# kzampog/cilantro

Hardware: AMD Instinct MI355X
Metric: ICP corr. pairs/sec (+ iterations/sec), synthetic uniform clouds (higher is better)
Workload: dtype f32 search / f64 accumulate+solve

## Files before the change

cilantro_amd/build.py:

```python
import os
import subprocess
import sys
from concurrent.futures import ThreadPoolExecutor

HERE = os.path.dirname(os.path.abspath(__file__))
CSRC = os.path.join(HERE, "csrc")
LIBDIR = os.path.join(HERE, "lib")
OBJDIR = os.path.join(HERE, "lib", "obj")
LIB = os.path.join(LIBDIR, "libcilantro_hip.so")
SOURCES = ["kernels.hip", "warm.hip", "epilogue.hip", "affine.hip", "feat_warm.hip", "extract.hip", "grid_build.hip", "grid_downsample.hip", "components.hip", "filters.hip", "kmeans.hip", "ransac.hip", "ransac_transform.hip", "knn.hip", "bidir.hip", "tie_build.hip", "c_api.hip", "icp_loop.hip", "multi.hip"]
HEADERS = ["internal.hpp", "ctx.hpp", "device_mem.hpp", "stateless.hpp", "ransac_sampling.hpp", "loop_policy.hpp", "grid_policy.hpp", "solve.hpp", "rccl_api.hpp", "search_device.hpp", "affine_device.hpp", os.path.join("..", "..", "include", "cilantro_hip", "c_api.h")]
HIPCC = os.environ.get("HIPCC", "/opt/rocm/bin/hipcc")
FLAGS = ["--offload-arch=gfx950", "-O3", "-std=c++17", "-fPIC", "-ffp-contract=off", "-Wall",
         "-Wno-unused-result", "-DNDEBUG"]
EXTRA_FLAGS = {f: ["-fno-slp-vectorize"] for f in ("kernels.hip", "warm.hip", "epilogue.hip", "affine.hip", "extract.hip")}


def _stale(out, deps):
    if not os.path.exists(out):
        return True
    t = os.path.getmtime(out)
    return any(os.path.getmtime(d) > t for d in deps)


def build(force=False, verbose=False, defines=(), tag=""):
    global OBJDIR, LIB
# ... 36 lines not shown
```

cilantro_amd/csrc/c_api.hip:

```cpp
#include <algorithm>
#include <chrono>
#include <cmath>
#include <cstddef>
#include <cstdio>
#include <cstring>
#include <new>

#include "ctx.hpp"
#include "stateless.hpp"

namespace cilhip {
hipStream_t ctx_stream(const cilhip_ctx* c) { return c->stream; }
double ctx_wait_us(const cilhip_ctx* c) { return c->wait_us; }
}

static void drop_src_grid(cilhip_ctx* c) {
  static_cast<SrcGridBufs&>(*c) = SrcGridBufs{};
  c->src_grid = GridDev{}; c->has_src_grid = false;
}
static void drop_feat_tie_tables(cilhip_ctx* c) {
  c->d_tief_leaf_slot.reset(); c->d_tief_nodes.reset();
}
static void drop_tie_tables(cilhip_ctx* c) {
  c->d_tie_leaf_slot.reset(); c->d_tie_nodes.reset();
// ... 13 lines not shown
  if (device < 0 || device >= ndev) return CILHIP_ERR_INVALID;
  cilhip_ctx* c = new (std::nothrow) cilhip_ctx();
  if (!c) return CILHIP_ERR_HIP;
  c->device = device;
  if (hipSetDevice(device) != hipSuccess || c->own_stream.create() != hipSuccess) {
    delete c;
    return CILHIP_ERR_HIP;
  }
  c->stream = c->own_stream;
  if (c->d_state.alloc(1) != hipSuccess || c->d_count.alloc(1) != hipSuccess ||
      c->d_defer_flag.alloc(1) != hipSuccess || hipMemset(c->d_defer_flag, 0, sizeof(uint32_t)) != hipSuccess ||
      c->d_unproven.alloc(128) != hipSuccess || hipMemset(c->d_unproven, 0, 128 * sizeof(uint32_t)) != hipSuccess ||
      c->d_ticket.alloc(1) != hipSuccess || hipMemset(c->d_ticket, 0, sizeof(unsigned int)) != hipSuccess ||
      hipHostMalloc(&c->h_feedback, sizeof(Feedback), hipHostMallocMapped | hipHostMallocCoherent) != hipSuccess ||
      hipHostGetDevicePointer(reinterpret_cast<void**>(&c->d_feedback), c->h_feedback, 0) != hipSuccess ||
      c->d_trace.alloc(RUN_TRACE_CAP) != hipSuccess || hipMemset(c->d_trace, 0, RUN_TRACE_CAP * sizeof(uint4)) != hipSuccess ||
      c->d_stage.alloc(REDUCE_STAGE_DOUBLES) != hipSuccess || c->d_sums.alloc(3 * SUMS_MAX) != hipSuccess) {
    delete c;
    return CILHIP_ERR_HIP;
  }
  if (hipMemset(c->d_state, 0, sizeof(IcpState)) != hipSuccess) { delete c; return CILHIP_ERR_HIP; }
  c->d_tie_counters = reinterpret_cast<unsigned int*>(reinterpret_cast<char*>(c->d_state.get()) + offsetof(IcpState, tie_counters));
  memcpy(c->sort_T, kIdentity16, sizeof(kIdentity16));
  memcpy(c->nn_T, kIdentity16, sizeof(kIdentity16));
  *out = c;
  return CILHIP_OK;
}

static void free_source(cilhip_ctx* c) {
  static_cast<SourceBufs&>(*c) = SourceBufs{};
  c->src_grid = GridDev{}; c->has_src_grid = false;
  c->rev_tie_valid = false; c->rev_tie_aware = false;
  c->src3_valid = false; c->lb_fresh = false; c->rec_valid = false;
  c->d_tiles = nullptr; c->d_tile_center = nullptr; c->ntiles = 0;
  c->has_source = false; c->src_sorted = false; drop_matches(c); c->ns = 0;
  c->have_pairs = false; c->pairs.count = 0;
// ... 192 lines not shown
#ifdef CILHIP_EXP_PHASE_CLOCKS
  cilhip::debug_dump_phase_clocks();
#endif
  return CILHIP_OK;
}

int cilhip_debug_live_allocations(unsigned long long out[2]) {
  if (!out) return CILHIP_ERR_INVALID;
  out[0] = dev_mem_live().count.load(std::memory_order_relaxed);
  out[1] = dev_mem_live().bytes.load(std::memory_order_relaxed);
  return CILHIP_OK;
}

int cilhip_get_last_timing2(cilhip_ctx* c, double* search_ms, double* accumulate_ms) {
  if (!c) return CILHIP_ERR_INVALID;
  if (search_ms) *search_ms = c->last_search_ms;
  if (accumulate_ms) *accumulate_ms = c->last_acc_ms;
  return CILHIP_OK;
}

int cilhip_get_last_iteration_timing(cilhip_ctx* c, int cap, int* n, unsigned int* iteration, float* kernel_ms) {
  if (!c || !n || cap < 0) return CILHIP_ERR_INVALID;
  const size_t m = c->timed_ms.size() < c->timed_iter.size() ? c->timed_ms.size() : c->timed_iter.size();
  *n = (int)m;
  for (size_t k = 0; k < m && k < (size_t)cap; ++k) { if (iteration) iteration[k] = c->timed_iter[k]; if (kernel_ms) kernel_ms[k] = c->timed_ms[k]; }
  return CILHIP_OK;
}

int cilhip_get_last_form_timing(cilhip_ctx* c, int form, double* kernel_ms, int* launches) {
  if (!c || form < 0 || form > 4) return CILHIP_ERR_INVALID;
  if (kernel_ms) *kernel_ms = c->form_ms[form];
  if (launches) *launches = c->form_n[form];
  return CILHIP_OK;
}

int cilhip_get_last_run_trace(cilhip_ctx* c, int cap, int* n_out, unsigned int* unproven, unsigned int* listed, float* step, float* delta, int* form) {
  if (!c || !n_out || cap < 0) return CILHIP_ERR_INVALID;
  CK(c, hipSetDevice(c->device));
  IcpState hs;
  CK(c, hipMemcpyAsync(&hs, c->d_state, sizeof(hs), hipMemcpyDeviceToHost, c->stream));
  uint4 tr[RUN_TRACE_CAP];
  CK(c, hipMemcpyAsync(tr, c->d_trace, sizeof(tr), hipMemcpyDeviceToHost, c->stream));
  CK(c, hipStreamSynchronize(c->stream));
  const int n = std::min(std::min(hs.iterations, (int)RUN_TRACE_CAP), cap);
  for (int i = 0; i < n; ++i) {
// ... 1411 lines not shown

int cilhip_get_grid_info(cilhip_ctx* c, cilhip_grid_info* o) {
  if (!c || !o) return CILHIP_ERR_INVALID;
  if (!c->has_target) return fail(c, CILHIP_ERR_INVALID, "no target");
  o->nx = c->grid.nx; o->ny = c->grid.ny; o->nz = c->grid.nz;
  o->cell = c->grid.cell;
  o->origin[0] = c->grid.ox; o->origin[1] = c->grid.oy; o->origin[2] = c->grid.oz;
  o->n_cells = c->grid_cells;
  o->avg_occupancy = c->grid_occ;
  o->build_ms = c->build_ms;
  return CILHIP_OK;
}

int cilhip_get_last_timing(cilhip_ctx* c, double* loop_ms, double* search_ms, int* launches) {
  if (!c) return CILHIP_ERR_INVALID;
  if (loop_ms) *loop_ms = c->last_loop_ms;
  if (search_ms) *search_ms = c->last_search_ms;
  if (launches) *launches = c->last_search_launches;
  return CILHIP_OK;
}
```

cilantro_amd/csrc/ctx.hpp:

```cpp
#pragma once

#include "../../include/cilantro_hip/c_api.h"

#include <hip/hip_runtime.h>

#include <string>
#include <vector>

#include "internal.hpp"
#include "loop_policy.hpp"

using namespace cilhip;

struct CtxStream { StreamGuard own_stream; };
struct TargetBufs {
  GridStore grid_store;
  SharedBuf<uint32_t> d_inv_perm;
  SharedBuf<uint2> d_tief_leaf_slot;
  SharedBuf<uint4> d_tief_nodes;
  SharedBuf<uint2> d_tie_leaf_slot;
  SharedBuf<uint4> d_tie_nodes;
  SharedBuf<float> d_safe2;
  DevBuf<unsigned long long> d_winner;
  DevBuf<float> d_dst_rgb;
// ... 44 lines not shown
  double build_ms = 0.0;
  float dst_mean[3] = {0, 0, 0};
  uint32_t index_offset = 0;
  bool partial_target = false;

  bool has_source = false;
  uint32_t ns = 0;
  uint2* d_tiles = nullptr;
  float4* d_tile_center = nullptr;
  float tile_axes[9] = {0, 0, 0, 0, 0, 0, 0, 0, 0};
  DevBuf<uint32_t> d_defer_flag;
  DevBuf<uint32_t> d_unproven;
  LoopPolicy policy;
  Feedback* h_feedback = nullptr;
  Feedback* d_feedback = nullptr;
  unsigned int run_tag = 0;
  int last_fused_iters = 0, last_two_pass_iters = 0, last_warm_iters = 0;
  int run_calls = 0;
  std::vector<unsigned char> iter_form;
  std::vector<unsigned char> trace_form;
  double form_ms[5] = {0, 0, 0, 0, 0};
  int form_n[5] = {0, 0, 0, 0, 0};
  int warm_start = 1;
  DevBuf<uint32_t> d_dbg;
  DevBuf<uint4> d_trace;
  uint32_t ntiles = 0;
  int tiled = 1;
  bool src_sorted = false;
  float sort_T[16];
  float src_mean[3] = {0, 0, 0};
// ... 70 lines not shown
  bool have_pairs = false;
  DevBuf<IcpState> d_state_id;

  cilhip_icp_params run_prm{};
  bool run_active = false;
  int guard_axis = -1;
  float guard_slack = 0.0f, guard_center[3] = {0, 0, 0}, guard_half[3] = {0, 0, 0}, guard_T[16] = {0};
  float run_src_mean[3] = {0, 0, 0};

  bool kernel_timing = false;
  int timing_stride = 1;
  std::vector<unsigned int> timed_iter;
  std::vector<float> timed_ms;
  double last_loop_ms = 0.0, last_search_ms = 0.0, last_acc_ms = 0.0;
  int last_search_launches = 0;
  size_t run_nev = 0;
  std::vector<hipEvent_t> ev, ev_acc;
  std::vector<hipEvent_t> ev_ar;
  size_t run_nar = 0;
  double last_allreduce_ms = 0.0; int last_allreduce_n = 0;
  double run_enqueue_us = 0.0; int run_enqueue_iters = 0;
};

inline cilhip_ctx::~cilhip_ctx() {
  if (h_feedback) (void)hipHostFree(h_feedback);
  for (auto e : ev) (void)hipEventDestroy(e);
  for (auto e : ev_acc) (void)hipEventDestroy(e);
  for (auto e : ev_ar) (void)hipEventDestroy(e);
}

#define CK(ctx, call)                                                                                   \
  do {                                                                                                  \
    hipError_t e_ = (call);                                                                             \
    if (e_ != hipSuccess) {                                                                             \
      (ctx)->err = std::string(#call) + ": " + hipGetErrorString(e_);                                   \
      return CILHIP_ERR_HIP;                                                                            \
    }                                                                                                   \
  } while (0)

namespace cilhip {
// ... 42 lines not shown
int ensure_safe2(cilhip_ctx* c);
int ensure_feature_arrays(cilhip_ctx* c);
int ensure_reverse_buffers(cilhip_ctx* c);
void set_warm_args(const cilhip_ctx* c, IterArgs& wa);
CorrWeights corr_weights_of(const cilhip_ctx* c, const cilhip_icp_params* p);
FeatSpec feat_spec_of(const cilhip_ctx* c);
TieDev tie_dev_rev(const cilhip_ctx* c);
int tie_prepare(cilhip_ctx* c, const char* what);
int tie_check_pending(cilhip_ctx* c, bool* again);
int apply_filters(cilhip_ctx* c);
IterArgs make_iter_args(cilhip_ctx* c, float max_sq);
int launch_search(cilhip_ctx* c, const IterArgs& a, int lanes = -1 );
int run_pair_search(cilhip_ctx* c, const IterArgs& a, float max_sq, const float T_host[16]);
int icp_run_affine(cilhip_ctx* c, const cilhip_icp_params* p, const float* T0, cilhip_icp_result* out);
int iter_metric_of(const cilhip_ctx* c, const cilhip_icp_params* p);
}
```

cilantro_amd/csrc/epilogue.hip:

```cpp
#include "search_device.hpp"
#include "affine_device.hpp"

namespace cilhip {

__device__ void reduce_partials_block(const double* __restrict__ partials, int nblocks, double* sums ) {
  __shared__ double sh[4][64];
  const int slot = threadIdx.x & 63, grp = threadIdx.x >> 6;
  double v = 0.0;
  if (slot < SUMS_MAX) {
    int b = grp;
    for (; b + 28 < nblocks; b += 32) {
      double r[8];
#pragma unroll
      for (int k = 0; k < 8; ++k) r[k] = partials[(size_t)(b + 4 * k) * SUMS_MAX + slot];
#pragma unroll
      for (int k = 0; k < 8; ++k) v += r[k];
    }
    for (; b < nblocks; b += 4) v += partials[(size_t)b * SUMS_MAX + slot];
  }
  sh[grp][slot] = v;
  __syncthreads();
  if (threadIdx.x < SUMS_MAX)
    sums[threadIdx.x] = (sh[0][threadIdx.x] + sh[1][threadIdx.x]) + (sh[2][threadIdx.x] + sh[3][threadIdx.x]);
  __syncthreads();
// ... 106 lines not shown

__device__ __forceinline__ void publish_state(const SolveArgs& a, const IcpState& lst) {
  if (a.trace != nullptr && a.gn_last_step && threadIdx.x == 0 && lst.iterations >= 1 && lst.iterations <= RUN_TRACE_CAP)
    a.trace[lst.iterations - 1] = make_uint4(lst.unproven, lst.listed, __float_as_uint(lst.motion_step), __float_as_uint(lst.delta));
  if (a.feedback != nullptr && a.gn_last_step && threadIdx.x == 0) {
    FeedbackSlot* sl = &a.feedback->slot[(unsigned int)lst.iterations & 3u];
    sl->unproven = lst.unproven;
    sl->listed = lst.listed;
    sl->delta = lst.delta;
    sl->prev_delta = lst.prev_delta;
    sl->step = lst.motion_step;
    sl->commit = ((unsigned long long)a.run_tag << 32) | (unsigned long long)(unsigned int)lst.iterations;
    __threadfence_system();
    a.feedback->latest = ((unsigned long long)a.run_tag << 32) | (lst.done ? 0x80000000ull : 0ull) | (unsigned long long)((unsigned int)lst.iterations & 0x7fffffffu);
  }
}

__device__ __forceinline__ void solve_body(const SolveArgs& a) {
  __shared__ double sums[SUMS_MAX];
  __shared__ IcpState lst;
  static_assert(sizeof(IcpState) % 4 == 0, "IcpState is copied as dwords");
  constexpr int ST_DWORDS = (int)(sizeof(IcpState) / 4);
  if (a.state->done) return;
  static_assert(ST_DWORDS <= 256, "one dword of the state per thread");
  const uint32_t sreg = (int)threadIdx.x < ST_DWORDS ? reinterpret_cast<const uint32_t*>(a.state)[threadIdx.x] : 0u;
  __shared__ unsigned int unproven_total;
  __shared__ unsigned int listed_total;
  const bool counters = a.unproven_cnt != nullptr && a.gn_last_step && threadIdx.x < 128;
  unsigned int cv = counters ? a.unproven_cnt[threadIdx.x] : 0u;
  if (a.nblocks > 0) {
// ... 61 lines not shown
        for (int r = 0; r < 3; ++r)
          t[r] = st->dtd[r] - (L[r * 3] * (double)st->smt[0] + L[r * 3 + 1] * (double)st->smt[1] + L[r * 3 + 2] * (double)st->smt[2]) +
                 (double)a.dst_mean[r];
      }
      finalize = true;
    }
  }
  if (finalize) {
    float Tn[16];
    const float delta = compose_update(L, t, st->T, Tn);
    finalize_state(st, a, Tn, delta);
  }
  }
  __syncthreads();
  for (int k = threadIdx.x; k < ST_DWORDS; k += 256) reinterpret_cast<uint32_t*>(a.state)[k] = reinterpret_cast<const uint32_t*>(&lst)[k];
  publish_state(a, lst);
}
__global__ __launch_bounds__(256) void k_solve(SolveArgs a) { solve_body(a); }

void launch_solve(const SolveArgs& a, hipStream_t s) {
  hipLaunchKernelGGL(k_solve, dim3(1), dim3(256), 0, s, a);
}

__global__ __launch_bounds__(256) void k_reduce_solve(const double* __restrict__ partials, int nblocks, double* __restrict__ stage, unsigned int* ticket, SolveArgs a) {
  if (a.state->done) return;
  {
    __shared__ double rsums[SUMS_MAX];
    const int per = (nblocks + (int)gridDim.x - 1) / (int)gridDim.x;
    const int b0 = blockIdx.x * per;
    const int b1 = min(b0 + per, nblocks);
// ... 212 lines not shown
    for (int r = 0; r < 3; ++r) dn = __fadd_rn(dn, __fmul_rn(dT[12 + r], dT[12 + r]));
    const float delta = sqrtf(dn);
    for (int i = 0; i < SUMS_MAX; ++i) st->sums[i] = 0.0;
    st->sums[0] = n;
    finalize_state(st, a, Tn, delta);
#ifdef CILHIP_EXP_AFF_CLOCKS
    {
      const unsigned long long c4_ = wall_clock64();
      st->unproven = (unsigned int)((c1_ - c0_) & 0xffffu) | (unsigned int)(((c2_ - c1_) & 0xffffu) << 16);
      st->listed = (unsigned int)((c3_ - c2_) & 0xffffu) | (unsigned int)(((c4_ - c3_) & 0xffffu) << 16);
    }
#endif
  }
  __syncthreads();
  for (int k = t; k < ST_DWORDS; k += NT) reinterpret_cast<uint32_t*>(a.state)[k] = reinterpret_cast<const uint32_t*>(&lst)[k];
  publish_state(a, lst);
}

void launch_reduce_and_solve_affine(const double* partials, int nrows, double* stage, const SolveArgs& a0, hipStream_t s) {
  SolveArgs a = a0;
  a.gn_last_step = 1;
  if (nrows > 64) {
    hipLaunchKernelGGL(k_reduce_affine, dim3(AFF_GROUPS), dim3(AFF_ROW), 0, s, partials, nrows, stage, (const IcpState*)a.state);
    a.partials = stage; a.nblocks = AFF_GROUPS;
  } else {
    a.partials = partials; a.nblocks = nrows;
  }
  a.reduced = nullptr;
  hipLaunchKernelGGL(k_solve_affine, dim3(1), dim3(AFF_SOLVE_THREADS), 0, s, a);
}
// ... 41 lines not shown
```

cilantro_amd/csrc/icp_loop.hip:

```cpp
#include <algorithm>
#include <chrono>
#include <cmath>
#include <cstddef>
#include <cstring>

#include "ctx.hpp"
#include "rccl_api.hpp"

int cilhip::iter_metric_of(const cilhip_ctx* c, const cilhip_icp_params* p) {
  if (p->metric == CILHIP_METRIC_POINT_TO_POINT) return IM_KABSCH;
  const bool wp = p->w_p2p > 0.0f, wl = p->w_p2pl > 0.0f;
  if (wl && !c->has_normals) return IM_POINT;
  if (wp && wl) return IM_BOTH;
  if (wl) return IM_PLANE;
  if (wp) return IM_POINT;
  return IM_PLANE;
}

static SolveArgs make_solve_args(cilhip_ctx* c, const cilhip_icp_params* p, int im, const float src_mean[3]) {
  SolveArgs sa{};
  sa.state = c->d_state;
  sa.partials = c->d_partials;
  sa.nblocks = iter_num_blocks(c->ns);
  sa.reduced = nullptr;
// ... 32 lines not shown
        v->unproven = sl->unproven; v->listed = sl->listed; v->delta = sl->delta; v->prev_delta = sl->prev_delta; v->step = iters ? sl->step : INFINITY;
        if (iters == 0u || sl->commit == (((unsigned long long)c->run_tag << 32) | iters)) return 0;
      }
    }
    cpu_relax(spins);
    if ((spins & 1023u) == 1023u && std::chrono::duration<double>(std::chrono::steady_clock::now() - t0).count() > patience_s) return 1;
  }
}
static int wait_published_or_sync(cilhip_ctx* c, unsigned int need, FbView* v) {
  if (wait_published(c, need, 30.0, v) == 0) return CILHIP_OK;
  CK(c, hipStreamSynchronize(c->stream));
  if (wait_published(c, need, 0.01, v) == 0) return CILHIP_OK;
  return fail(c, CILHIP_ERR_HIP, "icp_run: the device stopped publishing its loop state");
}

static int read_state(cilhip_ctx* c, cilhip_icp_result* out, float* Tprev = nullptr) {
  IcpState hs;
  CK(c, hipMemcpyAsync(&hs, c->d_state, sizeof(hs), hipMemcpyDeviceToHost, c->stream));
  CK(c, hipStreamSynchronize(c->stream));
  memcpy(c->tie_counters_host, hs.tie_counters, sizeof(c->tie_counters_host));
  c->tie_counters_fresh = true;
  memcpy(out->T, hs.T, sizeof(hs.T));
  if (Tprev) memcpy(Tprev, hs.Tprev, sizeof(hs.Tprev));
  out->iterations = (size_t)hs.iterations;
  out->last_delta_norm = hs.delta;
  out->last_ncorr = (size_t)hs.ncorr;
  return CILHIP_OK;
}

static void finish_run_matches(cilhip_ctx* c, const cilhip_icp_params* p, size_t iterations, const float Tprev[16], bool stored, bool pairs) {
  drop_matches(c); c->have_pairs = false;
  if (iterations == 0) return;
  memcpy(c->nn_T, Tprev, sizeof(c->nn_T));
  if (pairs) { c->have_pairs = true; c->matches_origin = 1; return; }
  if (stored && c->ns) {
    c->have_nn = true; c->d2_stale = true; c->matches_origin = 1;
  } else {
    c->pending_matches = true; c->pending_max_sq = p->max_sq_dist; c->matches_origin = 2;
  }
}

struct RunSetup {
  const cilhip_icp_params* p;
// ... 38 lines not shown
  launch_search_tiled(fa, im, c->d_tiles, c->d_tile_center, c->d_tile_box, c->ntiles, c->stream);
  c->rec_valid = recs; c->lb_fresh = false;
  return recs;
}

static int stop_when_done(cilhip_ctx* c, size_t it, size_t max_iter, bool* stop) {
  *stop = false;
  if (!(max_iter > 64 && (it + 1) % 32 == 0 && it + 1 < max_iter)) return CILHIP_OK;
  int done = 0;
  CK(c, hipMemcpyAsync(&done, reinterpret_cast<const char*>(c->d_state.get()) + offsetof(IcpState, done), sizeof(int), hipMemcpyDeviceToHost, c->stream));
  CK(c, hipStreamSynchronize(c->stream));
  *stop = done != 0;
  return CILHIP_OK;
}

static int finish_run(cilhip_ctx* c, const RunSetup& r, bool stored, bool pairs) {
  CK(c, hipEventRecord(r.e_end, c->stream));
  CK(c, hipGetLastError());
  float Tprev[16];
  const int rc = read_state(c, r.out, Tprev);
  if (rc) return rc;
  finish_run_matches(c, r.p, r.out->iterations, Tprev, stored, pairs && r.out->iterations > 0);
  float ms = 0.f;
  CK(c, hipEventElapsedTime(&ms, r.e_beg, r.e_end));
  c->last_loop_ms = ms; c->last_search_ms = 0.0; c->last_search_launches = 0;
  return CILHIP_OK;
}

static int run_reverse_loop(cilhip_ctx* c, RunSetup& r) {
  const cilhip_icp_params* p = r.p;
  IterArgs& a = r.a;
  SolveArgs& sa = r.sa;
  const int im = r.im;
  int rc = ensure_reverse_buffers(c);
  if (rc) return rc;
  FeatSpec rf = a.feat;
  rf.src = c->src_grid.nrm;
  if (rf.dst2) rf.src2 = c->d_src_rgb_grid;
  if (feat6(c) && (!rf.src || !rf.dst || (rf.dst2 && !rf.src2))) return fail(c, CILHIP_ERR_INVALID, "feature search: both clouds' feature vectors are needed");
  const int nb_f = iter_num_blocks(c->ns), nb_r = iter_num_blocks(c->grid.n);
  const bool fwd_wcap = c->search_dir == 2 && warm_capable(c);
// ... 51 lines not shown
      sa.reduced = nullptr;
      launch_solve(sa, c->stream);
    }
    bool stop = false;
    rc = stop_when_done(c, it, p->max_iter, &stop);
    if (rc) return rc;
    if (stop) break;
  }
  c->last_acc_ms = 0.0;
  return finish_run(c, r, false, false);
}

static int run_pair_list_loop(cilhip_ctx* c, RunSetup& r) {
  const cilhip_icp_params* p = r.p;
  SolveArgs& sa = r.sa;
  for (size_t it = 0; it < p->max_iter; ++it) {
    int rc = run_pair_search(c, r.a, p->max_sq_dist, it == 0 ? r.Ti : r.out->T);
    if (rc) return rc;
    IterArgs pa = r.a;
    pa.nn_d2 = c->pairs.d2;
    pa.src = c->pairs.src_view; pa.src_nrm = (c->d_src_nrm && c->symmetric) ? c->pairs.nrm_view : nullptr; pa.ns = c->pairs.count; pa.nn_pos = c->pairs.posd;
    const int pnb = iter_num_blocks(pa.ns);
    rc = ensure_partial_rows(c, (size_t)pnb);
    if (rc) return rc;
    pa.partials = c->d_partials;
    for (size_t st = 0; st < r.opt_steps; ++st) {
      pa.skip_if_inner_done = (st > 0);
      sa.gn_last_step = (st + 1 == r.opt_steps);
      if (pa.ns) {
        launch_iter(pa, r.im, false, false, pnb, c->stream);
// ... 152 lines not shown
    }
    sa.gn_last_step = (st + 1 == opt_steps);
    if (c->ns) {
      const int prows = (st == 0 && warm) ? warm_num_blocks(c->ns) : (st == 0 && one_pass) ? tiled_partial_rows(c->ntiles) : (st == 0 && feat_fused_it) ? feat_warm_blocks(c->ns)
                        : r.affine ? r.nb_aff : nb;
      if (r.affine) launch_reduce_and_solve_affine(c->d_partials, prows, c->d_stage, sa, c->stream);
      else launch_reduce_and_solve(c->d_partials, prows, c->d_stage, c->fused_epilogue ? c->d_ticket : nullptr, sa, c->stream);
    } else {
      launch_solve(sa, c->stream);
    }
  }
  f.prev_stored = stored_now && c->ns != 0;
  return CILHIP_OK;
}

static int collect_kernel_timing(cilhip_ctx* c, const ForwardRun& f, size_t iterations) {
  size_t executed = 0;
  while (executed < c->timed_iter.size() && (size_t)c->timed_iter[executed] < iterations) ++executed;
  c->last_acc_ms = 0.0;
  c->timed_ms.assign(executed, 0.0f);
  for (size_t k = 0; k < executed; ++k) {
    float m = 0.f;
    CK(c, hipEventElapsedTime(&m, c->ev[2 + 2 * k], c->ev[3 + 2 * k]));
    c->timed_ms[k] = m;
    c->last_search_ms += m;
    if (k < c->iter_form.size()) { c->form_ms[c->iter_form[k]] += m; ++c->form_n[c->iter_form[k]]; }
  }
  for (size_t k = 0; k + 1 < f.nacc; k += 2) {
    float m = 0.f;
    CK(c, hipEventElapsedTime(&m, c->ev_acc[k], c->ev_acc[k + 1]));
    c->last_acc_ms += m;
  }
  c->last_search_launches = (int)executed;
  return CILHIP_OK;
}

static int run_forward_loop(cilhip_ctx* c, RunSetup& r) {
  const cilhip_icp_params* p = r.p;
  IterArgs& a = r.a;
  int rc;
  if (feat6(c)) { rc = ensure_feature_arrays(c); if (rc) return rc; a.feat = feat_spec_of(c); }
  if (!filters_active(c) && !(a.cw.enabled && feat6(c))) a.nn_d2 = nullptr;
  ForwardRun f{};
// ... 5 lines not shown
  f.fwcap = feat6(c) && c->feat_warm && c->warm_start != 0 && c->ns >= 400000 && !filters_active(c) && !c->fused && !r.affine;
  if (f.fwcap) {
    rc = ensure_safe2(c); if (rc) return rc;
    rc = grow_partials(c, r, (size_t)feat_warm_blocks(c->ns)); if (rc) return rc;
  }
  f.paced = ((f.tile_acc || f.wcap) && c->ns && p->max_iter > 2 && c->tile_acc_adaptive) || (f.fwcap && p->max_iter > 2);
  if (f.tile_acc && !c->tile_acc_adaptive) c->policy.far_mode = false;
  c->last_fused_iters = c->last_two_pass_iters = c->last_warm_iters = 0;
  c->rec_valid = false; c->lb_fresh = false;
  c->policy.begin_run(c->warm_enter * c->grid.cell);
  c->iter_form.clear(); c->trace_form.clear(); c->timed_iter.clear();
  for (int k = 0; k < 5; ++k) { c->form_ms[k] = 0.0; c->form_n[k] = 0; }
  f.glanes = c->group_lanes > 0 ? c->group_lanes
             : (c->group_lanes < 0 && !use_tiled(c) && !feat6(c) && !c->fused) ? (c->ns <= 400000u ? 16 : c->ns <= 1500000u ? 8 : 0) : 0;
  f.group_now = f.glanes != 0 && (c->group_lanes > 0 || !f.wcap);
  for (size_t it = 0; it < p->max_iter; ++it) {
    bool stop = false;
    if (f.paced) { rc = pace_forward(c, f, it, &stop); if (rc) return rc; if (stop) break; }
    const bool one_pass = f.tile_acc && !c->policy.far_mode;
    const bool warm = f.wcap && it >= 1 && (c->warm_start == 2 || (f.paced && c->policy.on));
    const bool timing_it = f.timing && (c->timing_stride <= 1 || it < 3 || it % (size_t)c->timing_stride == 0);
    rc = enqueue_forward_iteration(c, r, f, it, one_pass, warm, timing_it);
    if (rc) return rc;
    if (!f.paced) { rc = stop_when_done(c, it, p->max_iter, &stop); if (rc) return rc; if (stop) break; }
  }
  rc = finish_run(c, r, f.all_stored && !filters_active(c) && !feat6(c), false);
  if (rc) return rc;
#ifdef CILHIP_EXP_PHASE_CLOCKS
  cilhip::debug_dump_phase_clocks();
#endif
  return f.timing ? collect_kernel_timing(c, f, r.out->iterations) : CILHIP_OK;
}

static int icp_run_once(cilhip_ctx* c, const cilhip_icp_params* p, const float* T0, cilhip_icp_result* out) {
  if (c->weight_fn && p->metric == CILHIP_METRIC_COMBINED && c->transform_mode == 0) {
    if (c->search_dir != 0) return fail(c, CILHIP_ERR_UNSUPPORTED, "a pair-weight callback runs with SECOND_TO_FIRST searches (rigid loop); estimate from pair lists through cilhip_estimate_combined");
    c->last_loop_ms = 0.0; c->last_search_ms = 0.0; c->last_acc_ms = 0.0; c->last_search_launches = 0;
    return cilhip_icp_run_two_sets(c, p->max_sq_dist, c, p->max_sq_dist, p, T0, out);
  }
  RunSetup r{};
  r.p = p; r.out = out;
  r.affine = c->transform_mode == 1;
  if (r.affine) {
    if (c->index_offset) return fail(c, CILHIP_ERR_UNSUPPORTED, "the affine variants are not available on target shards");
    const bool device_loop = c->affine_device_loop && c->ns != 0 && c->grid.n != 0 && c->search_dir == 0 && !filters_active(c) && !weighted(c) && !feat6(c) && !c->fused &&
                             !(c->d_src_nrm && c->symmetric) && c->guard_axis < 0;
    if (!device_loop) return icp_run_affine(c, p, T0, out);
  }
  r.Ti = T0 ? T0 : kIdentity16;
  int rc = ensure_sorted(c, r.Ti);
  if (rc) return rc;
  const bool affine_combined = r.affine && p->metric == CILHIP_METRIC_COMBINED;
  r.im = !r.affine ? iter_metric_of(c, p) : (affine_combined && p->w_p2pl > 0.0f && c->has_normals) ? IM_AFFC : IM_AFFP;
  r.gn = (r.im != IM_KABSCH) && !r.affine;
  const bool zero_steps = r.gn && p->max_opt_iter == 0;
  r.opt_steps = r.gn ? (p->max_opt_iter ? p->max_opt_iter : 1) : 1;
  ++c->run_tag;
  launch_init_state(c->d_state, r.Ti, c->src_mean, c->stream, c->d_feedback, c->run_tag, c->src_center, c->src_half, c->d_tie_counters);
  if (r.gn && c->ns >= 65536) ensure_pair_records(c);
  r.a = make_iter_args(c, p->max_sq_dist);
  if (!c->pair_records) r.a.grid.pn = nullptr;
  r.a.cw = corr_weights_of(c, p);
  r.sa = make_solve_args(c, p, r.im, c->src_mean);
  r.sa.gn_zero_steps = zero_steps ? 1 : 0;
  r.nb = r.sa.nblocks;
  r.nb_aff = r.affine ? affine_acc_blocks(c->ns) : 0;
  if (r.affine) {
    r.a.no_centering = affine_combined ? 0 : 1;
    r.sa.affine_centered = affine_combined ? 1 : 0;
    if (!affine_combined) { r.sa.w_p2p = 1.0f; r.sa.w_p2pl = 0.0f; }
    const size_t rows = (size_t)std::max(r.nb_aff, warm_num_blocks(c->ns));
    rc = grow_partials(c, r, (rows * AFF_ROW + SUMS_MAX - 1) / SUMS_MAX);
    if (rc) return rc;
  }
  if (c->ns == 0) {
    CK(c, hipMemsetAsync(c->d_sums, 0, SUMS_MAX * sizeof(double), c->stream));
    r.sa.nblocks = 0;
    r.sa.reduced = c->d_sums;
  }
  r.e_beg = event_at(c->ev, 0); r.e_end = event_at(c->ev, 1);
  return c->search_dir != 0 ? run_other_directions(c, r) : run_forward_loop(c, r);
}

int cilhip_icp_run(cilhip_ctx* c, const cilhip_icp_params* p, const float* T0, cilhip_icp_result* out) {
  if (!c || !p || !out) return CILHIP_ERR_INVALID;
  if (p->metric != CILHIP_METRIC_POINT_TO_POINT && p->metric != CILHIP_METRIC_COMBINED) return fail(c, CILHIP_ERR_INVALID, "icp_run: bad metric");
  CK(c, hipSetDevice(c->device));
  int rc = tie_prepare(c, "icp_run");
  if (rc) return rc;
  rc = icp_run_once(c, p, T0, out);
  if (rc) return rc;
  bool again = false;
  rc = tie_check_pending(c, &again);
  if (rc) return rc;
  return again ? icp_run_once(c, p, T0, out) : CILHIP_OK;
}

int cilhip_icp_begin(cilhip_ctx* c, const cilhip_icp_params* p, const float* T0, const float* gmean) {
  if (!c || !p) return CILHIP_ERR_INVALID;
  CK(c, hipSetDevice(c->device));
  if (p->metric == CILHIP_METRIC_COMBINED && p->max_opt_iter != 1) return fail(c, CILHIP_ERR_UNSUPPORTED, "sharded runs support max_opt_iter == 1");
  if (filters_active(c)) return fail(c, CILHIP_ERR_UNSUPPORTED, "inlier_fraction / one_to_one are global filters: not available in sharded runs");
  if (c->weight_fn && p->metric == CILHIP_METRIC_COMBINED)
    return fail(c, CILHIP_ERR_UNSUPPORTED, "a pair-weight callback is evaluated on the host, per estimate: not available in sharded runs (the stock evaluators are)");
  { const int trc = tie_prepare(c, "icp_begin"); if (trc) return trc; }
  if (c->search_dir != 0) return fail(c, CILHIP_ERR_UNSUPPORTED, "search directions other than SECOND_TO_FIRST are not available in sharded runs");
  if (feat6(c) || c->transform_mode != 0) return fail(c, CILHIP_ERR_UNSUPPORTED, "point+normal features and the affine variants are not available in sharded runs");
  const float* Ti = T0 ? T0 : kIdentity16;
  int rc = ensure_sorted(c, Ti);
  if (rc) return rc;
  c->run_prm = *p;
  for (int i = 0; i < 3; ++i) c->run_src_mean[i] = gmean ? gmean[i] : c->src_mean[i];
  ++c->run_tag;
  launch_init_state(c->d_state, Ti, c->run_src_mean, c->stream, c->d_feedback, c->run_tag, c->src_center, c->src_half, c->d_tie_counters);
  CK(c, hipGetLastError());
  c->run_active = true;
  c->run_nev = 0; c->run_nar = 0; c->last_allreduce_ms = 0.0; c->last_allreduce_n = 0;
  c->run_enqueue_us = 0.0; c->run_enqueue_iters = 0;
  c->run_calls = 0;
  c->rec_valid = false; c->lb_fresh = false;
  c->policy.begin_run(c->warm_enter * c->grid.cell);
  if (warm_capable(c) && !(c->d_src_nrm && c->symmetric)) { rc = ensure_safe2(c); if (rc) return rc; rc = ensure_warm_buffers(c); if (rc) return rc; }
  c->iter_form.clear(); c->trace_form.clear();
  for (int k = 0; k < 5; ++k) { c->form_ms[k] = 0.0; c->form_n[k] = 0; }
  c->last_fused_iters = c->last_two_pass_iters = c->last_warm_iters = 0;
  return CILHIP_OK;
}

// ... 207 lines not shown
```

cilantro_amd/csrc/internal.hpp:

```cpp
#pragma once

#include <hip/hip_runtime.h>
#include <stdint.h>

#include <string>
#include <thread>

#include "device_mem.hpp"
#include "grid_policy.hpp"
#include "solve.hpp"

struct cilhip_ctx;

namespace cilhip {

constexpr uint32_t NONE_U32 = 0xFFFFFFFFu;
#ifndef CILHIP_CUBE_EDGE
#define CILHIP_CUBE_EDGE 12
#endif
constexpr int CUBE_EDGE = CILHIP_CUBE_EDGE;
#ifndef CILHIP_TILE_THREADS
#define CILHIP_TILE_THREADS 1024
#endif
#ifndef CILHIP_TILE_WAVES_PER_SIMD
// ... 138 lines not shown
};

struct FeedbackSlot {
  unsigned int unproven;
  unsigned int listed;
  float delta;
  float prev_delta;
  float step;
  float pad;
  unsigned long long commit;
};
struct Feedback {
  FeedbackSlot slot[4];
  unsigned long long latest;
};

struct SolveArgs {
  Feedback* feedback;
  unsigned int run_tag;
  IcpState* state;
  const double* partials;
  int nblocks;
  const double* reduced;
  int metric;
  float w_p2p, w_p2pl;
  int point_weighted;
  float conv_tol, opt_conv_tol;
  float dst_mean[3], src_mean[3];
  int gn_last_step;
  int gn_zero_steps;
  int has_normals;
  int affine_centered;
  uint32_t* unproven_cnt;
  int guard_axis;
  float guard_slack;
  float guard_center[3], guard_half[3];
  float guard_T[16];
  float src_center[3], src_half[3];
  uint4* trace;
};
constexpr int RUN_TRACE_CAP = 256;

#if defined(__HIPCC__)
__device__ __forceinline__ bool tie_before(const TieDev& tt, float qx, float qy, float qz, uint32_t pa, uint32_t pb) {
  const uint2 la = tt.leaf_slot[pa], lb = tt.leaf_slot[pb];
  if (la.x == lb.x) return la.y < lb.y;
  uint32_t na = la.x, nb = lb.x;
  uint4 A = tt.nodes[na], B = tt.nodes[nb];
  uint32_t a_second = 0;
  while ((A.y >> 3) > (B.y >> 3)) { a_second = A.y & 1u; na = A.x; A = tt.nodes[na]; }
  while ((B.y >> 3) > (A.y >> 3)) { nb = B.x; B = tt.nodes[nb]; }
  while (na != nb) { a_second = A.y & 1u; na = A.x; A = tt.nodes[na]; nb = B.x; B = tt.nodes[nb]; }
  const uint32_t feat = (A.y >> 1) & 3u;
  const float val = feat == 0u ? qx : (feat == 1u ? qy : qz);
// ... 171 lines not shown
```

Before: 108.5 billion.

## Publish final ICP state to mapped host memory and defer timing readout

The solve kernel now writes the final IcpState into a host-mapped coherent image with a commit word. The host polls that image instead of issuing a device-to-host memcpy plus a stream synchronize. Event-based timing collection is deferred until a timing getter is called, which removes event syncs from the run's critical path. The cost is a system-scope fence and extra host-visible writes in the final solve, plus fallback paths if the image is not committed in time.

```diff
diff --git a/cilantro_amd/build.py b/cilantro_amd/build.py
--- a/cilantro_amd/build.py
+++ b/cilantro_amd/build.py
@@ -9,7 +9,7 @@
 OBJDIR = os.path.join(HERE, "lib", "obj")
 LIB = os.path.join(LIBDIR, "libcilantro_hip.so")
 SOURCES = ["kernels.hip", "warm.hip", "epilogue.hip", "affine.hip", "feat_warm.hip", "extract.hip", "grid_build.hip", "grid_downsample.hip", "components.hip", "filters.hip", "kmeans.hip", "ransac.hip", "ransac_transform.hip", "knn.hip", "bidir.hip", "tie_build.hip", "c_api.hip", "icp_loop.hip", "multi.hip"]
-HEADERS = ["internal.hpp", "ctx.hpp", "device_mem.hpp", "stateless.hpp", "ransac_sampling.hpp", "loop_policy.hpp", "grid_policy.hpp", "solve.hpp", "rccl_api.hpp", "search_device.hpp", "affine_device.hpp", os.path.join("..", "..", "include", "cilantro_hip", "c_api.h")]
+HEADERS = ["internal.hpp", "ctx.hpp", "device_mem.hpp", "stateless.hpp", "ransac_sampling.hpp", "loop_policy.hpp", "state_image.hpp", "grid_policy.hpp", "solve.hpp", "rccl_api.hpp", "search_device.hpp", "affine_device.hpp", os.path.join("..", "..", "include", "cilantro_hip", "c_api.h")]
 HIPCC = os.environ.get("HIPCC", "/opt/rocm/bin/hipcc")
 FLAGS = ["--offload-arch=gfx950", "-O3", "-std=c++17", "-fPIC", "-ffp-contract=off", "-Wall",
          "-Wno-unused-result", "-DNDEBUG"]
diff --git a/cilantro_amd/csrc/c_api.hip b/cilantro_amd/csrc/c_api.hip
--- a/cilantro_amd/csrc/c_api.hip
+++ b/cilantro_amd/csrc/c_api.hip
@@ -3,6 +3,7 @@
 #include <cmath>
 #include <cstddef>
 #include <cstdio>
+#include <cstdlib>
 #include <cstring>
 #include <new>
 
@@ -51,12 +52,16 @@
       c->d_ticket.alloc(1) != hipSuccess || hipMemset(c->d_ticket, 0, sizeof(unsigned int)) != hipSuccess ||
       hipHostMalloc(&c->h_feedback, sizeof(Feedback), hipHostMallocMapped | hipHostMallocCoherent) != hipSuccess ||
       hipHostGetDevicePointer(reinterpret_cast<void**>(&c->d_feedback), c->h_feedback, 0) != hipSuccess ||
+      hipHostMalloc(&c->h_image, sizeof(StateImage), hipHostMallocMapped | hipHostMallocCoherent) != hipSuccess ||
+      hipHostGetDevicePointer(reinterpret_cast<void**>(&c->d_image), c->h_image, 0) != hipSuccess ||
       c->d_trace.alloc(RUN_TRACE_CAP) != hipSuccess || hipMemset(c->d_trace, 0, RUN_TRACE_CAP * sizeof(uint4)) != hipSuccess ||
       c->d_stage.alloc(REDUCE_STAGE_DOUBLES) != hipSuccess || c->d_sums.alloc(3 * SUMS_MAX) != hipSuccess) {
     delete c;
     return CILHIP_ERR_HIP;
   }
   if (hipMemset(c->d_state, 0, sizeof(IcpState)) != hipSuccess) { delete c; return CILHIP_ERR_HIP; }
+  memset(c->h_image, 0, sizeof(StateImage));
+  { const char* e = getenv("CILHIP_EXP_STATE_COPY"); c->state_copy = e && e[0] == '1'; }
   c->d_tie_counters = reinterpret_cast<unsigned int*>(reinterpret_cast<char*>(c->d_state.get()) + offsetof(IcpState, tie_counters));
   memcpy(c->sort_T, kIdentity16, sizeof(kIdentity16));
   memcpy(c->nn_T, kIdentity16, sizeof(kIdentity16));
@@ -279,6 +284,7 @@
 
 int cilhip_get_last_timing2(cilhip_ctx* c, double* search_ms, double* accumulate_ms) {
   if (!c) return CILHIP_ERR_INVALID;
+  { const int trc = settle_timing(c); if (trc) return trc; }
   if (search_ms) *search_ms = c->last_search_ms;
   if (accumulate_ms) *accumulate_ms = c->last_acc_ms;
   return CILHIP_OK;
@@ -286,6 +292,7 @@
 
 int cilhip_get_last_iteration_timing(cilhip_ctx* c, int cap, int* n, unsigned int* iteration, float* kernel_ms) {
   if (!c || !n || cap < 0) return CILHIP_ERR_INVALID;
+  { const int trc = settle_timing(c); if (trc) return trc; }
   const size_t m = c->timed_ms.size() < c->timed_iter.size() ? c->timed_ms.size() : c->timed_iter.size();
   *n = (int)m;
   for (size_t k = 0; k < m && k < (size_t)cap; ++k) { if (iteration) iteration[k] = c->timed_iter[k]; if (kernel_ms) kernel_ms[k] = c->timed_ms[k]; }
@@ -294,6 +301,7 @@
 
 int cilhip_get_last_form_timing(cilhip_ctx* c, int form, double* kernel_ms, int* launches) {
   if (!c || form < 0 || form > 4) return CILHIP_ERR_INVALID;
+  { const int trc = settle_timing(c); if (trc) return trc; }
   if (kernel_ms) *kernel_ms = c->form_ms[form];
   if (launches) *launches = c->form_n[form];
   return CILHIP_OK;
@@ -1735,6 +1743,7 @@
 
 int cilhip_get_last_timing(cilhip_ctx* c, double* loop_ms, double* search_ms, int* launches) {
   if (!c) return CILHIP_ERR_INVALID;
+  { const int trc = settle_timing(c); if (trc) return trc; }
   if (loop_ms) *loop_ms = c->last_loop_ms;
   if (search_ms) *search_ms = c->last_search_ms;
   if (launches) *launches = c->last_search_launches;
diff --git a/cilantro_amd/csrc/ctx.hpp b/cilantro_amd/csrc/ctx.hpp
--- a/cilantro_amd/csrc/ctx.hpp
+++ b/cilantro_amd/csrc/ctx.hpp
@@ -82,6 +82,9 @@
   LoopPolicy policy;
   Feedback* h_feedback = nullptr;
   Feedback* d_feedback = nullptr;
+  StateImage* h_image = nullptr;
+  StateImage* d_image = nullptr;
+  bool state_copy = false;
   unsigned int run_tag = 0;
   int last_fused_iters = 0, last_two_pass_iters = 0, last_warm_iters = 0;
   int run_calls = 0;
@@ -182,6 +185,12 @@
   std::vector<float> timed_ms;
   double last_loop_ms = 0.0, last_search_ms = 0.0, last_acc_ms = 0.0;
   int last_search_launches = 0;
+  struct TimingDebt {
+    bool loop = false;
+    bool kernels = false;
+    size_t nacc = 0;
+    size_t iterations = 0;
+  } timing_debt;
   size_t run_nev = 0;
   std::vector<hipEvent_t> ev, ev_acc;
   std::vector<hipEvent_t> ev_ar;
@@ -192,6 +201,7 @@
 
 inline cilhip_ctx::~cilhip_ctx() {
   if (h_feedback) (void)hipHostFree(h_feedback);
+  if (h_image) (void)hipHostFree(h_image);
   for (auto e : ev) (void)hipEventDestroy(e);
   for (auto e : ev_acc) (void)hipEventDestroy(e);
   for (auto e : ev_ar) (void)hipEventDestroy(e);
@@ -264,4 +274,5 @@
 int run_pair_search(cilhip_ctx* c, const IterArgs& a, float max_sq, const float T_host[16]);
 int icp_run_affine(cilhip_ctx* c, const cilhip_icp_params* p, const float* T0, cilhip_icp_result* out);
 int iter_metric_of(const cilhip_ctx* c, const cilhip_icp_params* p);
-}
+int settle_timing(cilhip_ctx* c);
+}
diff --git a/cilantro_amd/csrc/epilogue.hip b/cilantro_amd/csrc/epilogue.hip
--- a/cilantro_amd/csrc/epilogue.hip
+++ b/cilantro_amd/csrc/epilogue.hip
@@ -144,6 +144,17 @@
     __threadfence_system();
     a.feedback->latest = ((unsigned long long)a.run_tag << 32) | (lst.done ? 0x80000000ull : 0ull) | (unsigned long long)((unsigned int)lst.iterations & 0x7fffffffu);
   }
+}
+
+template <int NT>
+__device__ __forceinline__ void publish_image(const SolveArgs& a, const IcpState& lst) {
+  if (a.image == nullptr || a.feedback == nullptr || !a.gn_last_step) return;
+  if (!(lst.done || lst.iterations == a.max_iter)) return;
+  constexpr int ST_DWORDS = (int)(sizeof(IcpState) / 4);
+  for (int k = threadIdx.x; k < ST_DWORDS; k += NT) a.image->state[k] = reinterpret_cast<const uint32_t*>(&lst)[k];
+  if (threadIdx.x == 0) a.image->commit = ((unsigned long long)a.run_tag << 32) | (unsigned long long)(unsigned int)lst.iterations;
+  __threadfence_system();
+  __syncthreads();
 }
 
 __device__ __forceinline__ void solve_body(const SolveArgs& a) {
@@ -235,6 +246,7 @@
   }
   __syncthreads();
   for (int k = threadIdx.x; k < ST_DWORDS; k += 256) reinterpret_cast<uint32_t*>(a.state)[k] = reinterpret_cast<const uint32_t*>(&lst)[k];
+  publish_image<256>(a, lst);
   publish_state(a, lst);
 }
 __global__ __launch_bounds__(256) void k_solve(SolveArgs a) { solve_body(a); }
@@ -477,6 +489,7 @@
   }
   __syncthreads();
   for (int k = t; k < ST_DWORDS; k += NT) reinterpret_cast<uint32_t*>(a.state)[k] = reinterpret_cast<const uint32_t*>(&lst)[k];
+  publish_image<NT>(a, lst);
   publish_state(a, lst);
 }
 
diff --git a/cilantro_amd/csrc/icp_loop.hip b/cilantro_amd/csrc/icp_loop.hip
--- a/cilantro_amd/csrc/icp_loop.hip
+++ b/cilantro_amd/csrc/icp_loop.hip
@@ -6,6 +6,17 @@
 
 #include "ctx.hpp"
 #include "rccl_api.hpp"
+#include "state_image.hpp"
+
+#ifdef CILHIP_EXP_HOST_PHASES
+#include <cstdio>
+namespace { struct HostPhases { std::chrono::steady_clock::time_point t[6]; double w[2]; } g_hp; }
+#define HP_STAMP(i) (g_hp.t[i] = std::chrono::steady_clock::now())
+#define HP_WAIT(i, c) (g_hp.w[i] = (c)->wait_us)
+#else
+#define HP_STAMP(i) ((void)0)
+#define HP_WAIT(i, c) ((void)0)
+#endif
 
 int cilhip::iter_metric_of(const cilhip_ctx* c, const cilhip_icp_params* p) {
   if (p->metric == CILHIP_METRIC_POINT_TO_POINT) return IM_KABSCH;
@@ -70,10 +81,7 @@
   return fail(c, CILHIP_ERR_HIP, "icp_run: the device stopped publishing its loop state");
 }
 
-static int read_state(cilhip_ctx* c, cilhip_icp_result* out, float* Tprev = nullptr) {
-  IcpState hs;
-  CK(c, hipMemcpyAsync(&hs, c->d_state, sizeof(hs), hipMemcpyDeviceToHost, c->stream));
-  CK(c, hipStreamSynchronize(c->stream));
+static void state_to_result(cilhip_ctx* c, const IcpState& hs, cilhip_icp_result* out, float* Tprev) {
   memcpy(c->tie_counters_host, hs.tie_counters, sizeof(c->tie_counters_host));
   c->tie_counters_fresh = true;
   memcpy(out->T, hs.T, sizeof(hs.T));
@@ -81,8 +89,16 @@
   out->iterations = (size_t)hs.iterations;
   out->last_delta_norm = hs.delta;
   out->last_ncorr = (size_t)hs.ncorr;
-  return CILHIP_OK;
-}
+}
+
+static int read_state(cilhip_ctx* c, cilhip_icp_result* out, float* Tprev = nullptr) {
+  IcpState hs;
+  CK(c, hipMemcpyAsync(&hs, c->d_state, sizeof(hs), hipMemcpyDeviceToHost, c->stream));
+  CK(c, hipStreamSynchronize(c->stream));
+  state_to_result(c, hs, out, Tprev);
+  return CILHIP_OK;
+}
+
 
 static void finish_run_matches(cilhip_ctx* c, const cilhip_icp_params* p, size_t iterations, const float Tprev[16], bool stored, bool pairs) {
   drop_matches(c); c->have_pairs = false;
@@ -151,17 +167,42 @@
   return CILHIP_OK;
 }
 
+constexpr double FINISH_PATIENCE_S = 2.0e-3;
+
+static int take_final_state(cilhip_ctx* c, const RunSetup& r, float* Tprev) {
+  const size_t max_iter = r.p->max_iter;
+  if (max_iter == 0 || !r.sa.image || !r.sa.feedback || !c->h_image || !c->h_feedback) return read_state(c, r.out, Tprev);
+  FbView fv;
+  const unsigned int need = max_iter < 0x7fffffffu ? (unsigned int)max_iter : 0x7fffffffu;
+  if (wait_published(c, need, FINISH_PATIENCE_S, &fv) != 0) return read_state(c, r.out, Tprev);
+  HP_STAMP(3);
+  unsigned int iters = 0;
+  const unsigned long long latest = const_cast<const volatile Feedback*>(c->h_feedback)->latest;
+  IcpState hs;
+  static_assert(sizeof(hs) == sizeof(c->h_image->state), "the image is the state, dword for dword");
+  if (!latest_is_final(latest, c->run_tag, (unsigned long long)max_iter, &iters) ||
+      !take_state_image(c->h_image->state, &c->h_image->commit, sizeof(IcpState) / 4, offsetof(IcpState, iterations) / 4, c->run_tag, iters,
+                        reinterpret_cast<uint32_t*>(&hs)))
+    return read_state(c, r.out, Tprev);
+  state_to_result(c, hs, r.out, Tprev);
+  return CILHIP_OK;
+}
+
 static int finish_run(cilhip_ctx* c, const RunSetup& r, bool stored, bool pairs) {
   CK(c, hipEventRecord(r.e_end, c->stream));
   CK(c, hipGetLastError());
   float Tprev[16];
-  const int rc = read_state(c, r.out, Tprev);
-  if (rc) return rc;
+#ifdef CILHIP_EXP_HOST_PHASES
+  if (!r.sa.image) { CK(c, hipStreamSynchronize(c->stream)); HP_STAMP(3); }
+#endif
+  const int rc = r.sa.image ? take_final_state(c, r, Tprev) : read_state(c, r.out, Tprev);
+  if (rc) return rc;
+  HP_STAMP(4);
   finish_run_matches(c, r.p, r.out->iterations, Tprev, stored, pairs && r.out->iterations > 0);
-  float ms = 0.f;
-  CK(c, hipEventElapsedTime(&ms, r.e_beg, r.e_end));
-  c->last_loop_ms = ms; c->last_search_ms = 0.0; c->last_search_launches = 0;
-  return CILHIP_OK;
+  c->last_loop_ms = 0.0; c->last_search_ms = 0.0; c->last_search_launches = 0;
+  c->timing_debt = cilhip_ctx::TimingDebt{};
+  c->timing_debt.loop = true;
+  return c->state_copy ? settle_timing(c) : CILHIP_OK;
 }
 
 static int run_reverse_loop(cilhip_ctx* c, RunSetup& r) {
@@ -243,6 +284,7 @@
 static int run_pair_list_loop(cilhip_ctx* c, RunSetup& r) {
   const cilhip_icp_params* p = r.p;
   SolveArgs& sa = r.sa;
+  sa.image = nullptr;
   for (size_t it = 0; it < p->max_iter; ++it) {
     int rc = run_pair_search(c, r.a, p->max_sq_dist, it == 0 ? r.Ti : r.out->T);
     if (rc) return rc;
@@ -425,9 +467,20 @@
   return CILHIP_OK;
 }
 
-static int collect_kernel_timing(cilhip_ctx* c, const ForwardRun& f, size_t iterations) {
+int cilhip::settle_timing(cilhip_ctx* c) {
+  const cilhip_ctx::TimingDebt d = c->timing_debt;
+  if (!d.loop && !d.kernels) return CILHIP_OK;
+  c->timing_debt = cilhip_ctx::TimingDebt{};
+  CK(c, hipSetDevice(c->device));
+  CK(c, hipEventSynchronize(c->ev[1]));
+  if (d.loop) {
+    float ms = 0.f;
+    CK(c, hipEventElapsedTime(&ms, c->ev[0], c->ev[1]));
+    c->last_loop_ms = ms;
+  }
+  if (!d.kernels) return CILHIP_OK;
   size_t executed = 0;
-  while (executed < c->timed_iter.size() && (size_t)c->timed_iter[executed] < iterations) ++executed;
+  while (executed < c->timed_iter.size() && (size_t)c->timed_iter[executed] < d.iterations) ++executed;
   c->last_acc_ms = 0.0;
   c->timed_ms.assign(executed, 0.0f);
   for (size_t k = 0; k < executed; ++k) {
@@ -437,7 +490,7 @@
     c->last_search_ms += m;
     if (k < c->iter_form.size()) { c->form_ms[c->iter_form[k]] += m; ++c->form_n[c->iter_form[k]]; }
   }
-  for (size_t k = 0; k + 1 < f.nacc; k += 2) {
+  for (size_t k = 0; k + 1 < d.nacc; k += 2) {
     float m = 0.f;
     CK(c, hipEventElapsedTime(&m, c->ev_acc[k], c->ev_acc[k + 1]));
     c->last_acc_ms += m;
@@ -473,6 +526,7 @@
   f.glanes = c->group_lanes > 0 ? c->group_lanes
              : (c->group_lanes < 0 && !use_tiled(c) && !feat6(c) && !c->fused) ? (c->ns <= 400000u ? 16 : c->ns <= 1500000u ? 8 : 0) : 0;
   f.group_now = f.glanes != 0 && (c->group_lanes > 0 || !f.wcap);
+  HP_STAMP(1); HP_WAIT(0, c);
   for (size_t it = 0; it < p->max_iter; ++it) {
     bool stop = false;
     if (f.paced) { rc = pace_forward(c, f, it, &stop); if (rc) return rc; if (stop) break; }
@@ -483,15 +537,20 @@
     if (rc) return rc;
     if (!f.paced) { rc = stop_when_done(c, it, p->max_iter, &stop); if (rc) return rc; if (stop) break; }
   }
+  HP_STAMP(2); HP_WAIT(1, c);
   rc = finish_run(c, r, f.all_stored && !filters_active(c) && !feat6(c), false);
   if (rc) return rc;
 #ifdef CILHIP_EXP_PHASE_CLOCKS
   cilhip::debug_dump_phase_clocks();
 #endif
-  return f.timing ? collect_kernel_timing(c, f, r.out->iterations) : CILHIP_OK;
+  if (f.timing) { c->timing_debt.kernels = true; c->timing_debt.nacc = f.nacc; c->timing_debt.iterations = r.out->iterations; }
+  rc = c->state_copy ? settle_timing(c) : CILHIP_OK;
+  HP_STAMP(5);
+  return rc;
 }
 
 static int icp_run_once(cilhip_ctx* c, const cilhip_icp_params* p, const float* T0, cilhip_icp_result* out) {
+  c->timing_debt = cilhip_ctx::TimingDebt{};
   if (c->weight_fn && p->metric == CILHIP_METRIC_COMBINED && c->transform_mode == 0) {
     if (c->search_dir != 0) return fail(c, CILHIP_ERR_UNSUPPORTED, "a pair-weight callback runs with SECOND_TO_FIRST searches (rigid loop); estimate from pair lists through cilhip_estimate_combined");
     c->last_loop_ms = 0.0; c->last_search_ms = 0.0; c->last_acc_ms = 0.0; c->last_search_launches = 0;
@@ -521,6 +580,7 @@
   if (!c->pair_records) r.a.grid.pn = nullptr;
   r.a.cw = corr_weights_of(c, p);
   r.sa = make_solve_args(c, p, r.im, c->src_mean);
+  if (!c->state_copy) { r.sa.image = c->d_image; r.sa.max_iter = p->max_iter < 0x7fffffffu ? (int)p->max_iter : 0x7fffffff; }
   r.sa.gn_zero_steps = zero_steps ? 1 : 0;
   r.nb = r.sa.nblocks;
   r.nb_aff = r.affine ? affine_acc_blocks(c->ns) : 0;
@@ -545,10 +605,22 @@
   if (!c || !p || !out) return CILHIP_ERR_INVALID;
   if (p->metric != CILHIP_METRIC_POINT_TO_POINT && p->metric != CILHIP_METRIC_COMBINED) return fail(c, CILHIP_ERR_INVALID, "icp_run: bad metric");
   CK(c, hipSetDevice(c->device));
+#ifdef CILHIP_EXP_HOST_PHASES
+  HP_STAMP(0); for (int k = 1; k < 6; ++k) g_hp.t[k] = g_hp.t[0];
+  g_hp.w[0] = g_hp.w[1] = c->wait_us;
+#endif
   int rc = tie_prepare(c, "icp_run");
   if (rc) return rc;
   rc = icp_run_once(c, p, T0, out);
   if (rc) return rc;
+#ifdef CILHIP_EXP_HOST_PHASES
+  {
+    auto us = [](int a, int b) { return std::chrono::duration<double, std::micro>(g_hp.t[b] - g_hp.t[a]).count(); };
+    const double lw = g_hp.w[1] - g_hp.w[0];
+    std::fprintf(stderr, "[host phases] ns=%u max_iter=%zu iters=%zu path=%s us: setup %.1f enqueue %.1f wait %.1f (loop %.1f + finish %.1f) state_read %.1f timing_readout %.1f total %.1f\n",
+                 c->ns, (size_t)p->max_iter, out->iterations, c->state_copy ? "copy" : "image", us(0, 1), us(1, 2) - lw, lw + us(2, 3), lw, us(2, 3), us(3, 4), us(4, 5), us(0, 5));
+  }
+#endif
   bool again = false;
   rc = tie_check_pending(c, &again);
   if (rc) return rc;
@@ -571,6 +643,7 @@
   c->run_prm = *p;
   for (int i = 0; i < 3; ++i) c->run_src_mean[i] = gmean ? gmean[i] : c->src_mean[i];
   ++c->run_tag;
+  c->timing_debt = cilhip_ctx::TimingDebt{};
   launch_init_state(c->d_state, Ti, c->run_src_mean, c->stream, c->d_feedback, c->run_tag, c->src_center, c->src_half, c->d_tie_counters);
   CK(c, hipGetLastError());
   c->run_active = true;
diff --git a/cilantro_amd/csrc/internal.hpp b/cilantro_amd/csrc/internal.hpp
--- a/cilantro_amd/csrc/internal.hpp
+++ b/cilantro_amd/csrc/internal.hpp
@@ -176,6 +176,10 @@
   FeedbackSlot slot[4];
   unsigned long long latest;
 };
+struct StateImage {
+  uint32_t state[sizeof(IcpState) / 4];
+  unsigned long long commit;
+};
 
 struct SolveArgs {
   Feedback* feedback;
@@ -200,6 +204,8 @@
   float guard_T[16];
   float src_center[3], src_half[3];
   uint4* trace;
+  StateImage* image;
+  int max_iter;
 };
 constexpr int RUN_TRACE_CAP = 256;
 
diff --git a/cilantro_amd/csrc/state_image.hpp b/cilantro_amd/csrc/state_image.hpp
--- /dev/null
+++ b/cilantro_amd/csrc/state_image.hpp
@@ -0,0 +1,33 @@
+#pragma once
+
+#include <atomic>
+#include <cstddef>
+#include <cstdint>
+
+namespace cilhip {
+
+inline unsigned long long state_commit_word(unsigned int run_tag, unsigned int iterations) {
+  return ((unsigned long long)run_tag << 32) | (unsigned long long)iterations;
+}
+
+inline bool take_state_image(const volatile uint32_t* image, const volatile unsigned long long* commit, size_t n, size_t iter_dword,
+                             unsigned int run_tag, unsigned int iterations, uint32_t* out) {
+  if (image == nullptr || commit == nullptr || out == nullptr || iter_dword >= n) return false;
+  const unsigned long long want = state_commit_word(run_tag, iterations);
+  if (*commit != want) return false;
+  std::atomic_thread_fence(std::memory_order_acquire);
+  for (size_t k = 0; k < n; ++k) out[k] = image[k];
+  std::atomic_thread_fence(std::memory_order_acquire);
+  if (*commit != want) return false;
+  return out[iter_dword] == iterations;
+}
+
+inline bool latest_is_final(unsigned long long latest, unsigned int run_tag, unsigned long long max_iter, unsigned int* iterations) {
+  if ((unsigned int)(latest >> 32) != run_tag) return false;
+  const unsigned int iters = (unsigned int)latest & 0x7fffffffu;
+  if (iterations) *iterations = iters;
+  const bool done = (latest & 0x80000000ull) != 0ull;
+  return iters >= 1u && (done || (unsigned long long)iters == max_iter);
+}
+
+}
```

Measured after the change: 108.5 billion, median of 3. Within noise of the previous version (+0.0%).
